# king159/Pair-Net

Hardware: AMD Instinct MI355X
Metric: images/sec (whole node), 100-query 800x1333, 1/2/4/8 MI355X (higher is better)
Workload: dtype f32

## Files before the change

### include/pairnet_hip.h

```cpp
#ifndef PAIRNET_HIP_H_
#define PAIRNET_HIP_H_

#include <stdint.h>

#ifdef __cplusplus
extern "C" {
#endif

#define PN_ABI_VERSION 33
int pn_abi_version(void);

#define PN_GEMM_RELU       1
#define PN_GEMM_A_COLMAJOR 2
#define PN_GEMM_FORCE_TILE 4
#define PN_GEMM_FORCE_SKINNY 8
#define PN_GEMM_FORCE_TILE64 16
#define PN_GEMM_FORCE_TILE128x64 32
#define PN_GEMM_RELU_AFTER_RES 128
#define PN_GEMM_GELU 256
#define PN_GEMM_RESERVE_SHIFT 16
#define PN_GEMM_RESERVE(n) ((((n) / 8) & 0x3ff) << PN_GEMM_RESERVE_SHIFT)
#define PN_GEMM_KSPLIT_SHIFT 26
#define PN_GEMM_KSPLIT(n) (((n) & 31) << PN_GEMM_KSPLIT_SHIFT)

// ... 140 lines not shown
                         int64_t out_bstride, void* stream);
int pn_bilinear_planar_f32(const float* in, float* out, int64_t P, int hi,
                           int wi, int ho, int wo, void* stream);
int pn_bilinear_stencil_rows_f32(const float* in, float* out, int B, int hi, int wi, int ho,
                                 int wo, int C, int64_t in_bstride, int64_t out_bstride,
                                 void* stream);
int pn_bilinear_planar_gt0_u8(const float* in, uint8_t* out, int64_t P, int hi,
                              int wi, int ho, int wo, void* stream);

int pn_mask_pack(const float* logits, uint32_t* bits, int32_t* rowall,
                 int64_t R, int Nk, void* stream);
int pn_mask_pack_stencil(const float* logits4, uint32_t* bits, int32_t* rowall, int64_t R,
                         int hi, int wi, int ho, int wo, void* stream);

int pn_mask_stencil_gemm_f32(const float* me, int64_t ld_me, int64_t stride_me, const float* rows,
                             int64_t ld_rows, int64_t stride_rows, uint32_t* bits,
                             int32_t* rowall, int B, int Q, int Nk, int K, int hi, int wi, int ho,
                             int wo, int flags, void* stream);

int pn_mask_stencil_gather_gemm_f32(const float* me, int64_t ld_me, int64_t stride_me,
                                    const float* mf, int64_t ld_mf, int64_t stride_mf,
                                    uint32_t* bits, int32_t* rowall, int B, int Q, int Nk, int K,
                                    int hi, int wi, int ho, int wo, int flags, void* stream);

int64_t pn_attn_scratch_floats(int B, int Q, int Nk);
int pn_attention_f32(const float* q, int64_t ldq, const float* k, int64_t ldk,
                     const float* v, int64_t ldv, const uint32_t* maskbits,
                     const int32_t* rowall, float* out, int64_t ldo,
                     float* scratch, int B, int Q, int Nk, float scale,
                     void* stream);

int pn_mlearner_first_f32(const float* in, const float* w1, const float* b1,
                          float* out, int B, int S, int C, void* stream);
int pn_ppn_front_f32(const float* sub_embed, const float* obj_embed, const float* w1,
                     const float* b1, float* importance_raw, float* c1, int B, int Q, float eps,
                     void* stream);
int pn_mlearner_last_f32(const float* in, const float* w3, const float* b3,
                         float* out, int B, int S, int C, void* stream);

int pn_topk_pairs(const float* scores, int64_t* idx, int64_t* sub, int64_t* obj,
                  int64_t* pair, int B, int Q, int k, void* stream);
int pn_topk_f32(const float* scores, int64_t* idx, int64_t* quot, int64_t* rem, int B,
                int n, int div, int k, void* stream);
int pn_topk_strided_f32(const float* scores, int64_t elem_stride, int64_t row_stride,
                        int64_t* idx, int64_t* quot, int64_t* rem, int B, int n, int div, int k,
                        void* stream);
// ... 221 lines not shown
```

### pair-net_amd/csrc/gemm.hip

```cpp
#include "common.h"
#include "gemm_common.h"

#ifndef PN_GEMM_WGS64
#define PN_GEMM_WGS64 5
#endif
#ifndef PN_GEMM_WGS128x64
#define PN_GEMM_WGS128x64 3
#endif
#ifndef PN_GEMM_BIGM_128x64
#define PN_GEMM_BIGM_128x64 0
#endif
#ifndef PN_GEMM_WGS64_SPILLING
#define PN_GEMM_WGS64_SPILLING 5
#endif

#ifndef PN_GEMM_LDS2
#define PN_GEMM_LDS2 0
#endif

template <int BM, int BN, int AMODE>
struct TileSmem {
  static constexpr int A_ELEMS = (AMODE == A_COL) ? 32 * (BM + 4) : BM * 36;
  static constexpr int STAGE = A_ELEMS + BN * 36;
  static constexpr int FLOATS = STAGE * (PN_GEMM_LDS2 ? 2 : 1);
// ... 14 lines not shown
  static constexpr int min_waves = (BM * BN <= 64 * 64 && value > 4) ? value : 1;
};

struct TileRef {
  int pi;
  int bz, tm, tn;
};

template <int BM, int BN, int WM, int WN, int AMODE, bool ADD, typename Locator, int EPI = 0>
__device__ __forceinline__ void gemm_persistent(const Locator& loc, const int ntiles,
                                                float* smem) {
  constexpr int BK = 32, LD = BK + 4;
  constexpr int WAVES_N = BN / WN;
  constexpr int TM = WM / 32, TN = WN / 32;
  constexpr int LDK = BM + 4;
  constexpr int A_ELEMS = TileSmem<BM, BN, AMODE>::A_ELEMS;
  constexpr int NT = 64 * (BM / WM) * WAVES_N;
  constexpr int RPP = NT / 8;
  constexpr int NA = (BM * BK / 4) / NT;
  constexpr int NB = (BN * BK / 4) / NT;
  constexpr int QM = BM / 4;
  constexpr int KSTEP = NT / QM;
  static_assert(NT == 128 || NT == 256 || NT == 512, "2, 4 or 8 waves");

  const int xcd = blockIdx.x & 7, slot = blockIdx.x >> 3, per = gridDim.x >> 3;
  const int q8 = ntiles >> 3, r8 = ntiles & 7;
  const int base = (xcd < r8) ? xcd * (q8 + 1) : r8 * (q8 + 1) + (xcd - r8) * q8;
  const int cnt = q8 + (xcd < r8 ? 1 : 0);
  if (slot >= cnt) return;

  const int tid = threadIdx.x, lane = tid & 63, wave = tid >> 6;
  const int li = lane & 31, lh = lane >> 5;
  const int wm = wave / WAVES_N, wn = wave % WAVES_N;
  const int kc = (tid & 7) * 4;
  float* const sA = smem;
  float* const sB = smem + A_ELEMS;

  int lpi = 0, lK = 0, lkt0 = 0;
  const float* bA = nullptr;
  const float* bW = nullptr;
  const float* bAdd = nullptr;
  __amdgpu_buffer_rsrc_t rA = make_rsrc(nullptr), rW = rA, rAdd = rA;
  unsigned a_off[NA], add_off[ADD ? NA : 1], w_off[NB];
  int cy[NA], cx[NA];
  unsigned a_tap[AMODE == A_CONV ? NA : 1];
  unsigned a_off1[AMODE == A_COL ? NA : 1][4];
// ... 21 lines not shown
#pragma unroll
      for (int j = 0; j < NA; ++j) {
        const unsigned krow = (unsigned)(min(tid / QM + KSTEP * j, p.K - 1)) * (unsigned)p.lda;
        a_off[j] = (krow + (unsigned)min(mq, p.M - 1)) * 4u;
#pragma unroll
        for (int e = 0; e < 4; ++e) a_off1[j][e] = (krow + (unsigned)min(mq + e, p.M - 1)) * 4u;
      }
    } else {
#pragma unroll
      for (int j = 0; j < NA; ++j) {
        const int gm = min(m0 + (tid >> 3) + RPP * j, p.M - 1);
        if (AMODE == A_CONV) {
          const int oy = gm / p.Wo, ox = gm - oy * p.Wo;
          cy[j] = oy * p.stride;
          cx[j] = ox * p.stride;
          a_off[j] = ((unsigned)(cy[j] * p.Wd + cx[j]) * (unsigned)p.Cin + kc) * 4u;
        } else {
          a_off[j] = ((unsigned)gm * (unsigned)p.lda + kc) * 4u;
        }
        if (ADD) add_off[j] = ((unsigned)(p.Aadd ? gm % p.aadd_rows : gm) *
                                   (unsigned)(p.Aadd ? p.ldaadd : p.lda) + kc) * 4u;
      }
    }
    if constexpr (EPI == 1 || EPI == 3) {
      const StencilP& st = loc.st;
#pragma unroll
      for (int j = 0; j < NB; ++j) {
        const int c = (tid >> 3) + RPP * j;
        const int key = min(tr.tn * 16 + (c >> 5) * 8 + (c & 7), st.nk - 1);
        if constexpr (EPI == 3) {
          const int t = (c >> 3) & 3;
          const int oy = key / st.wo, ox = key - oy * st.wo;
          const Tap ty = make_tap(oy, st.hi, st.ho), tx = make_tap(ox, st.wi, st.wo);
          const int sy = (t & 2) ? ty.i1 : ty.i0, sx = (t & 1) ? tx.i1 : tx.i0;
          w_off[j] = ((unsigned)(sy * st.wi + sx) * (unsigned)p.ldw + kc) * 4u;
        } else {
          w_off[j] = ((unsigned)(((c >> 3) & 3) * st.nk + key) * (unsigned)p.ldw + kc) * 4u;
        }
      }
    } else {
#pragma unroll
      for (int j = 0; j < NB; ++j)
        w_off[j] = ((unsigned)min(n0 + (tid >> 3) + RPP * j, p.N - 1) * (unsigned)p.ldw + kc) * 4u;
    }
  };

  float4 ra[NA], rad[ADD ? NA : 1], rb[NB];
  bool st_ragged = false, st_add = false;
  int st_k0 = 0;
  unsigned st_in = 0;
  auto load_chunk = [&](int kt) {
    const int k0 = (lkt0 + kt) * BK;
    const bool ragged = k0 + BK > lK;
    st_ragged = ragged;
    st_add = l_add;
    st_k0 = k0;
    if (AMODE == A_COL) {
      const GemmP& p = loc.P(lpi);
      const int soff = (ragged ? 0 : k0) * (int)p.lda * 4;
      if (l_vec) {
// ... 105 lines not shown
      if (AMODE == A_COL) {
        const float* s = fA + (kb * 8) * LDK + mi * 32;
        fa[mi] = make_float4(s[0], s[LDK], s[2 * LDK], s[3 * LDK]);
      } else {
        fa[mi] = ld4(fA + mi * 32 * LD + kb * 8);
      }
    }
#pragma unroll
    for (int ni = 0; ni < TN; ++ni) fb[ni] = ld4(fB + ni * 32 * LD + kb * 8);
  };
  auto compute = [&]() {
    float4 fa[2][TM], fb[2][TN];
    read_frag(0, fa[0], fb[0]);
#pragma unroll
    for (int kb = 0; kb < BK / 8; ++kb) {
      const int cur = kb & 1;
      if (kb + 1 < BK / 8) read_frag(kb + 1, fa[cur ^ 1], fb[cur ^ 1]);
#pragma unroll
      for (int t = 0; t < 4; ++t)
#pragma unroll
        for (int mi = 0; mi < TM; ++mi)
#pragma unroll
          for (int ni = 0; ni < TN; ++ni) {
            const float4 av = fa[cur][mi], bv = fb[cur][ni];
            acc[mi][ni] = mfma32(t == 0 ? av.x : t == 1 ? av.y : t == 2 ? av.z : av.w,
                                 t == 0 ? bv.x : t == 1 ? bv.y : t == 2 ? bv.z : bv.w,
                                 acc[mi][ni]);
          }
    }
  };

  static_assert(EPI != 2 || (TM == 1 && TN == 1 && !PN_GEMM_LDS2), "two-phase mode: 32x32 waves, one LDS stage");
  float keep[EPI == 2 ? 16 : 1];
  TileRef cur = loc(base + slot);
  set_tile(cur);
  load_chunk(0);
#if PN_GEMM_LDS2
  constexpr int STAGE = TileSmem<BM, BN, AMODE>::STAGE;
  int wso = 0;
  {
    const GemmP& p0 = loc.P(cur.pi);
    int nk0 = (p0.K + BK - 1) / BK;
    if (p0.ksplit > 1) nk0 = min(p0.split_chunks, nk0 - (cur.bz % p0.ksplit) * p0.split_chunks);
    store_chunk(0);
    wso = STAGE;
    if (nk0 > 1) {
      load_chunk(1);
// ... 35 lines not shown
          load_chunk(1);
        } else {
          set_tile(loc(base + min(t + 2 * per, cnt - 1)));
          load_chunk(0);
        }
      }
      compute();
      __syncthreads();
      rso = wso;
      wso = STAGE - wso;
    }
#else
    for (int kt = 0; kt < nk; ++kt) {
      __syncthreads();
      store_chunk();
      __syncthreads();
      const bool last = kt + 1 == nk;
      if (last) set_tile(nxt);
      load_chunk(last ? 0 : kt + 1);
      compute();
    }
#endif
    const int m0 = cur.tm * BM, n0 = cur.tn * BN;
    if constexpr (EPI == 1 || EPI == 3) {
      const StencilP& st = loc.st;
      static_assert((EPI != 1 && EPI != 3) || (TM == 1 && TN == 1 && BN == 64), "stencil mode: 64x64 tiles of 32x32 waves");
      const int pl = li & 7;
      const int key0 = cur.tn * 16 + wn * 8;
      const int key = key0 + pl;
      const bool kvalid = key < st.nk;
      const int kk = min(key, st.nk - 1);
      const int oy = kk / st.wo, ox = kk - oy * st.wo;
      const Tap ty = make_tap(oy, st.hi, st.ho), tx = make_tap(ox, st.wi, st.wo);
      const int src = (lane & 32) | pl;
      const int nwords = (st.nk + 31) / 32;
      const int nvalid = min(max(st.nk - key0, 0), 8);
      const unsigned vm = (1u << nvalid) - 1u;
      const int rbase = m0 + wm * WM;
      const bool writer = li == 0;
      const bool last_tile = (cur.tn + 1) * 16 >= st.nk && wn == WAVES_N - 1;
#pragma unroll
      for (int r = 0; r < 16; ++r) {
        const float a = acc[0][0][r];
        const float v00 = __shfl(a, src, 64), v01 = __shfl(a, src + 8, 64);
        const float v10 = __shfl(a, src + 16, 64), v11 = __shfl(a, src + 24, 64);
        const float res = tap_blend(ty, tx, v00, v01, v10, v11);
// ... 101 lines not shown
  const StencilP& st;
  int mt, nt;
  __device__ __forceinline__ const GemmP& P(int) const { return p; }
  __device__ __forceinline__ TileRef operator()(int T) const {
    const int per_b = mt * nt;
    const int bz = T / per_b, r = T - bz * per_b;
    const int tm = r / nt;
    return TileRef{0, bz, tm, r - tm * nt};
  }
};

__global__ __launch_bounds__(256, (TileWgs<64, 64, A_ROW, false>::min_waves))
void k_gemm_stencil(const GemmP p, const StencilP st, const int batch) {
  __shared__ __attribute__((aligned(16))) float smem[TileSmem<64, 64, A_ROW>::FLOATS];
  const StencilLocator loc{p, st, (p.M + 63) / 64, (p.N + 63) / 64};
  gemm_persistent<64, 64, 32, 32, A_ROW, false, StencilLocator, 1>(loc, loc.mt * loc.nt * batch, smem);
}

__global__ __launch_bounds__(256, (TileWgs<64, 64, A_ROW, false>::min_waves))
void k_gemm_stencil_gather(const GemmP p, const StencilP st, const int batch) {
  __shared__ __attribute__((aligned(16))) float smem[TileSmem<64, 64, A_ROW>::FLOATS];
  const StencilLocator loc{p, st, (p.M + 63) / 64, (p.N + 63) / 64};
  gemm_persistent<64, 64, 32, 32, A_ROW, false, StencilLocator, 3>(loc, loc.mt * loc.nt * batch, smem);
}

#define PN_GEMM_WGS_PROJ PN_GEMM_WGS64
struct ProjLocator {
  const GemmP& p;
  const GemmP& sc;
  int mt, nt;
  __device__ __forceinline__ const GemmP& P(int phase) const { return phase ? p : sc; }
  __device__ __forceinline__ TileRef operator()(int T) const {
    const int per_b = mt * nt;
    const int bz = T / per_b, r = T - bz * per_b;
    const int tm = r / nt;
    return TileRef{0, bz, tm, r - tm * nt};
  }
};

__global__ __launch_bounds__(256, PN_GEMM_WGS_PROJ)
void k_gemm_proj(const GemmP p, const GemmP sc, const int batch) {
  __shared__ __attribute__((aligned(16))) float smem[TileSmem<64, 64, A_CONV>::FLOATS];
  const ProjLocator loc{p, sc, (p.M + 63) / 64, (p.N + 63) / 64};
  gemm_persistent<64, 64, 32, 32, A_CONV, false, ProjLocator, 2>(loc, loc.mt * loc.nt * batch, smem);
}

// ... 456 lines not shown
  if (fused) {
    GemmP both = p3;
    both.K = Cin + planes;
    fused = splitk_factor(both, B, splitk_scratch, splitk_scratch_floats, &cps, flags) <= 1;
  }
  if (!fused) {
    if (!idt) return PN_BAD_ARG;
    if (stride == 1) {
      if (int rc = pn_gemm_f32(&ds, stream)) return rc;
    } else if (int rc = pn_conv2d_nhwc_ex_f32(x, Wsc, bsc, nullptr, idt, B, H, W, Cin, Cout, 1, 1,
                                              stride, 0, flags, splitk_scratch,
                                              splitk_scratch_floats, stream)) {
      return rc;
    }
    return pn_gemm_f32(&d3, stream);
  }
  const int64_t ntiles = (int64_t)pn_cdiv((int)M, 64) * pn_cdiv(Cout, 64) * B;
  static const int wgs = resident_wgs(k_gemm_proj, PN_GEMM_WGS_PROJ, 256);
  hipLaunchKernelGGL(k_gemm_proj, dim3(persistent_grid(ntiles, wgs, flags)), dim3(256), 0, s, p3,
                     psc, B);
  return PN_LAUNCH_CHECK();
}

extern "C" int pn_mask_stencil_gemm_f32(const float* me, int64_t ld_me, int64_t stride_me,
                                        const float* rows, int64_t ld_rows, int64_t stride_rows,
                                        uint32_t* bits, int32_t* rowall, int B, int Q, int Nk,
                                        int K, int hi, int wi, int ho, int wo, int flags,
                                        void* stream) {
  if (!me || !rows || !bits || !rowall || B <= 0 || Q <= 0 || Nk <= 0 || K <= 0 || K % 32)
    return PN_BAD_ARG;
  if (hi <= 0 || wi <= 0 || ho <= 0 || wo <= 0 || (int64_t)ho * wo != Nk) return PN_BAD_ARG;
  if (ld_me % 4 || ld_rows % 4 || stride_me % 4 || stride_rows % 4 || !aligned16(me) || !aligned16(rows))
    return PN_BAD_ARG;
  const int64_t lim = (int64_t)1 << 29;
  if ((int64_t)(Q - 1) * ld_me + K >= lim || ((int64_t)4 * Nk - 1) * ld_rows + K >= lim)
    return PN_BAD_ARG;
  GemmP p{};
  p.A = me; p.W = rows; p.lda = ld_me; p.ldw = ld_rows; p.sA = stride_me; p.sW = stride_rows;
  p.M = Q; p.K = K; p.aadd_rows = 1;
  p.N = pn_cdiv(Nk, 16) * 64;
  const StencilP st{bits, rowall, Nk, hi, wi, ho, wo};
  hipStream_t s = (hipStream_t)stream;
  hipLaunchKernelGGL(k_fill_i32, dim3(pn_cdiv(B * Q, 256)), dim3(256), 0, s, rowall, 1, B * Q);
  const int64_t ntiles = (int64_t)pn_cdiv(Q, 64) * (p.N / 64) * B;
  static const int wgs = resident_wgs(k_gemm_stencil, TileWgs<64, 64, A_ROW, false>::value, 256);
  hipLaunchKernelGGL(k_gemm_stencil, dim3(persistent_grid(ntiles, wgs, flags)), dim3(256), 0, s, p, st, B);
  return PN_LAUNCH_CHECK();
}

extern "C" int pn_mask_stencil_gather_gemm_f32(const float* me, int64_t ld_me, int64_t stride_me,
                                               const float* mf, int64_t ld_mf, int64_t stride_mf,
                                               uint32_t* bits, int32_t* rowall, int B, int Q,
                                               int Nk, int K, int hi, int wi, int ho, int wo,
                                               int flags, void* stream) {
  if (!me || !mf || !bits || !rowall || B <= 0 || Q <= 0 || Nk <= 0 || K <= 0 || K % 32)
    return PN_BAD_ARG;
  if (hi <= 0 || wi <= 0 || ho <= 0 || wo <= 0 || (int64_t)ho * wo != Nk) return PN_BAD_ARG;
  if (ld_me % 4 || ld_mf % 4 || stride_me % 4 || stride_mf % 4 || !aligned16(me) || !aligned16(mf))
    return PN_BAD_ARG;
  const int64_t lim = (int64_t)1 << 29;
  if ((int64_t)(Q - 1) * ld_me + K >= lim || ((int64_t)hi * wi - 1) * ld_mf + K >= lim)
    return PN_BAD_ARG;
  GemmP p{};
  p.A = me; p.W = mf; p.lda = ld_me; p.ldw = ld_mf; p.sA = stride_me; p.sW = stride_mf;
  p.M = Q; p.K = K; p.aadd_rows = 1;
  p.N = pn_cdiv(Nk, 16) * 64;
  const StencilP st{bits, rowall, Nk, hi, wi, ho, wo};
  hipStream_t s = (hipStream_t)stream;
  hipLaunchKernelGGL(k_fill_i32, dim3(pn_cdiv(B * Q, 256)), dim3(256), 0, s, rowall, 1, B * Q);
  const int64_t ntiles = (int64_t)pn_cdiv(Q, 64) * (p.N / 64) * B;
  static const int wgs = resident_wgs(k_gemm_stencil_gather, TileWgs<64, 64, A_ROW, false>::value, 256);
  hipLaunchKernelGGL(k_gemm_stencil_gather, dim3(persistent_grid(ntiles, wgs, flags)), dim3(256), 0,
                     s, p, st, B);
  return PN_LAUNCH_CHECK();
}

extern "C" int pn_abi_version(void) { return PN_ABI_VERSION; }
```

### pair-net_amd/head.py

```python
import math
from collections import OrderedDict

import torch

from . import hip
from . import plans
from .plans import Arena, PlanCache, measure_bytes
from .config import ConfigDict

INSTANCE_OFFSET = 1000


def _decoder_param_shapes(prefix, num_layers, ffn_dim, out):
    for i in range(num_layers):
        p = "%s.layers.%d." % (prefix, i)
        for a in (0, 1):
            out[p + "attentions.%d.attn.in_proj_weight" % a] = (768, 256)
            out[p + "attentions.%d.attn.in_proj_bias" % a] = (768,)
            out[p + "attentions.%d.attn.out_proj.weight" % a] = (256, 256)
            out[p + "attentions.%d.attn.out_proj.bias" % a] = (256,)
        out[p + "ffns.0.layers.0.0.weight"] = (ffn_dim, 256)
        out[p + "ffns.0.layers.0.0.bias"] = (ffn_dim,)
        out[p + "ffns.0.layers.1.weight"] = (256, ffn_dim)
        out[p + "ffns.0.layers.1.bias"] = (256,)
# ... 79 lines not shown
                                                 transformer_decoder=transformer_decoder,
                                                 relation_decoder=relation_decoder))
        self.other_drop_rates.pop("relation_decoder.transformerlayers.ffn_cfgs.ffn_drop", None)
        self.test_cfg, self.train_cfg = test_cfg, train_cfg
        assert len(self.in_channels) == 4 and num_transformer_feat_level == 3
        assert num_obj_query <= 256 and num_rel_query <= 128
        self._params = OrderedDict(
            (k, torch.zeros(s)) for k, s in self.param_shapes().items())
        self.device = None
        self.w = None
        self._plans = PlanCache()
        self._arenas, self._post_arenas, self._consts, self._pe = {}, {}, {}, OrderedDict()
        self._dummies = {}
        self._post = OrderedDict()
        self._pan_jobs = []
        self.graph_after = 1
        self.exact_mask_order = True
        self.conv_algo = "winograd4"
        self.use_graphs = False
        self.grid_reserve = 0
        self.fuse_ppn_front = True
        self.fuse_mask_pack = True
        self.gather_mask_stencil = True
        self.fuse_lateral_upadd = False
        self.enc_fused_ln = ("proj", "ffn")
        self.group_input_convs = False
        self.gemm_arithmetic = "bf16x3"
        self.msda_s3_out = False
        self.init_weights()

    def param_shapes(self):
        s = OrderedDict()
        Q, R = self.num_obj_query, self.num_rel_query
        _decoder_param_shapes("relation_decoder", self.num_rel_layers, self.rel_ffn, s)
        s["rel_query_embed.weight"] = (R, 256)
        s["rel_query_embed2.weight"] = (2 * R, 256)
        s["rel_query_embed3.weight"] = (2 * R, 256)
        s["rel_query_feat.weight"] = (R, 256)
        for i, (ci, co) in enumerate(((1, 64), (64, 64), (64, 1))):
            s["update_importance.conv_layers.%d.0.weight" % i] = (co, ci, 7, 7)
            s["update_importance.conv_layers.%d.0.bias" % i] = (co,)
        pd = "pixel_decoder."
        for i in range(3):
            cin = self.in_channels[3 - i]
            s[pd + "input_convs.%d.conv.weight" % i] = (256, cin, 1, 1)
            s[pd + "input_convs.%d.conv.bias" % i] = (256,)
# ... 538 lines not shown
                 batch=pl.B, sA=Q * 256, sW=pl.HW2 * 256, sC=Q * pl.HW2)

    def _head_embed(self, q, pl, with_cls, full_mask, cls_out=None, mp_out=None, normed=False):
        w, B, Q = self.w, pl.B, self.num_obj_query
        cls_out = pl.cls if cls_out is None else cls_out
        mp_out = pl.MP if mp_out is None else mp_out
        if not normed:
            hip.layernorm(q, w["transformer_decoder.post_norm.weight"],
                          w["transformer_decoder.post_norm.bias"], pl.qn)
        if with_cls:
            hip.linear(pl.qn, w["cls_embed.weight"], w["cls_embed.bias"], cls_out.view(B * Q, -1))
        self._mlp3("mask_embed", pl.qn, pl.me, pl)
        if full_mask:
            self._mask_logits(pl.me, pl, mp_out)

    def _attn_mask(self, pl, lvl, mp=None, me=None):
        B, Q = pl.B, self.num_obj_query
        h, wd = pl.shapes[lvl]
        n = h * wd
        if self.exact_mask_order == "full":
            hip.bilinear_planar(pl.MP if mp is None else mp, pl.ML, B * Q, pl.hw2[0], pl.hw2[1],
                                h, wd)
        elif self.exact_mask_order and self.fuse_mask_pack:
            if self._gathers_stencil():
                hip.mask_stencil_gather_gemm(pl.me if me is None else me, pl.MF, pl.bits,
                                             pl.rowall, B, Q, pl.hw2[0], pl.hw2[1], h, wd)
            else:
                hip.mask_stencil_gemm(pl.me if me is None else me, pl.MFs[lvl], pl.bits,
                                      pl.rowall, B, Q, pl.hw2[0], pl.hw2[1], h, wd)
            return
        elif self.exact_mask_order:
            hip.gemm(pl.me if me is None else me, pl.MFs[lvl], pl.ML4, M=Q, N=4 * n, K=256,
                     lda=256, ldw=256, ldc=4 * n, batch=B, sA=Q * 256, sW=4 * n * 256,
                     sC=Q * 4 * n, force="tile64")
            hip.mask_pack_stencil(pl.ML4, pl.bits, pl.rowall, B * Q, pl.hw2[0], pl.hw2[1], h, wd)
            return
        else:
            hip.gemm(pl.me if me is None else me, pl.MFd[lvl], pl.ML, M=Q, N=n, K=256, lda=256,
                     ldw=256, ldc=n, batch=B, sA=Q * 256, sW=n * 256, sC=Q * n)
        hip.mask_pack(pl.ML, pl.bits, pl.rowall, B * Q, n)

    def _layer(self, pre, x, xpos, x1, x2, y, Qp, VQK, att, hbuf, Kp, ldk, Vp, ldv, Nk, B, nq,
               bits, rowall, scr, ffn, self_first=False, post=None, x_in=None):
        w = self.w
        scale = 1.0 / math.sqrt(32.0)
        ac = pre + "attentions.%d.attn." % (1 if self_first else 0)
        as_ = pre + "attentions.%d.attn." % (0 if self_first else 1)
        nc, ns = ("norms.1.", "norms.0.") if self_first else ("norms.0.", "norms.1.")

        def cross(src, dst):
            hip.linear(src, w[ac + "in_proj_weight"][:256], w[ac + "in_proj_bias"][:256], Qp,
                       aadd=xpos)
# ... 142 lines not shown
    def _check_feats(self, feats, img_metas):
        pv = getattr(self, "_packed_version", None)
        if self.w is not None and pv is not None and pv != self._weights_version():
            self._drop_weight_state()
        B = len(img_metas)
        assert len(feats) == 4 and all(f.shape[0] == B for f in feats)
        nchw = all(f.is_contiguous() for f in feats)
        nhwc = not nchw and all(f.is_contiguous(memory_format=torch.channels_last) for f in feats)
        for f, c in zip(feats, self.in_channels):
            if not f.is_cuda or f.dtype != torch.float32 or f.shape[1] != c or not (nchw or nhwc):
                raise RuntimeError("feats must be fp32 [B,C,H,W] device tensors with channels %s, "
                                   "all contiguous or all in channels_last memory format"
                                   % self.in_channels)
        if self.device is None:
            self.to(feats[0].device)
        shapes = [tuple(feats[3 - l].shape[-2:]) for l in range(3)]
        self._feats_nhwc = nhwc
        return B, shapes, tuple(feats[0].shape[-2:])

    def _run_stage(self, which, pl, feats=None):
        cfg = (self.exact_mask_order, self.conv_algo, self.fuse_ppn_front, self.grid_reserve,
               tuple(self.enc_fused_ln), self.group_input_convs,
               getattr(self, "fuse_mask_pack", True), self.gemm_arithmetic, self.msda_s3_out,
               getattr(self, "gather_mask_stencil", True), getattr(self, "fuse_lateral_upadd", False))
        if pl.graph_cfg != cfg:
            pl.graph_a = pl.graph_b = None
            pl.graphs_a = OrderedDict()
            pl.graph_c = PlanCache(self.POST_VIEWS)
            pl.graph_cfg = cfg
        cur = torch.cuda.current_stream(self.device)
        pl.streams[cur.cuda_stream] = cur
        try:
            self._run_stage_on(which, pl, feats, cur)
        finally:
            plans.note_use(cur)

    def _run_stage_on(self, which, pl, feats, cur):
        if which == "a":
            if not pl.pe_waited:
                if pl.pe_ready.query():
                    pl.pe_waited = True
                else:
                    cur.wait_event(pl.pe_ready)
            ptrs = tuple(f.data_ptr() for f in feats)
            ent = pl.graphs_a.get(ptrs)
            if ent is None:
# ... 323 lines not shown
```

### pair-net_amd/hip.py

```python
import contextlib
import ctypes as C
import os
import threading

import torch

from .build import LIB_PATH

LIB_PATH = os.environ.get("PAIRNET_LIB") or LIB_PATH

_i32, _i64, _f32, _vp = C.c_int32, C.c_int64, C.c_float, C.c_void_p

GEMM_RELU, GEMM_A_COLMAJOR, GEMM_FORCE_TILE, GEMM_FORCE_SKINNY = 1, 2, 4, 8
GEMM_GELU = 256
GEMM_FORCE_TILE64, GEMM_FORCE_TILE128x64 = 16, 32
GEMM_RELU_AFTER_RES = 128
GEMM_GROUP_MAX = 18


class GemmDesc(C.Structure):
    _fields_ = [("A", _vp), ("lda", _i64), ("strideA", _i64),
                ("Aadd", _vp), ("ldaadd", _i64), ("aadd_rows", _i32),
                ("aadd_from_col", _i32),
                ("W", _vp), ("ldw", _i64), ("strideW", _i64),
# ... 105 lines not shown
    "pn_window_attention_bwd_f32": (C.c_int, [_vp, _i64, _vp, _vp, _vp, _i64, _vp, _i64, _vp, _i64, _vp]
                                    + [_i32] * 7 + [_f32, _vp]),
    "pn_grad_norm_clip_f32": (C.c_int, [_vp, _i64, _f32, _f32, _vp, _vp, _vp]),
    "pn_adamw_f32": (C.c_int, [_vp, _vp, _vp, _vp, _i64, _vp, _vp, _vp, _i32, _f32, _f32, _f32, _f32,
                               _f32, _i32, _vp, _f32, _vp]),
    "pn_adamw_guarded_f32": (C.c_int, [_vp, _vp, _vp, _vp, _i64, _vp, _vp, _vp, _i32, _f32, _f32,
                                       _f32, _f32, _f32, _i32, _vp, _f32, _vp, _vp]),
    "pn_lsa_f32": (C.c_int, [_vp, _i64, _vp, _i32, _i64, _vp, _vp, _i64, _vp, _vp]),
    "pn_loss_targets": (C.c_int, [_vp] * 6 + [_i64, _i32, _i32, _i32, _i32] + [_vp] * 5),
    "pn_msda_loc_f32": (C.c_int, [_vp, _i64, _vp, _vp, _vp, _vp, _vp, _i32, _i32, _i32, _i32, _vp]),
    "pn_msda_bwd_f32": (C.c_int, [_vp, _i64] + [_vp] * 8 + [_i32, _i32, _i32, _i32, _vp]),
    "pn_gather_probe_f32": (C.c_int, [_vp, _vp, _vp, _i32, _i32, _vp]),
    "pn_sine_pe_f32": (C.c_int, [_vp, _vp, _i32, _i32, _i32, _f32, _vp]),
    "pn_sine_pe_offset_f32": (C.c_int, [_vp, _vp, _i32, _i32, _i32, _f32, _f32, _vp]),
    "pn_bilinear_nhwc_f32": (C.c_int, [_vp, _vp] + [_i32] * 7 + [_i64, _i64, _vp]),
    "pn_bilinear_planar_f32": (C.c_int, [_vp, _vp, _i64] + [_i32] * 4 + [_vp]),
    "pn_bilinear_planar_gt0_u8": (C.c_int, [_vp, _vp, _i64] + [_i32] * 4 + [_vp]),
    "pn_mask_pack": (C.c_int, [_vp, _vp, _vp, _i64, _i32, _vp]),
    "pn_mask_pack_stencil": (C.c_int, [_vp, _vp, _vp, _i64, _i32, _i32, _i32, _i32, _vp]),
    "pn_mask_stencil_gemm_f32": (C.c_int, [_vp, _i64, _i64, _vp, _i64, _i64, _vp, _vp] +
                                 [_i32] * 9 + [_vp]),
    "pn_mask_stencil_gather_gemm_f32": (C.c_int, [_vp, _i64, _i64, _vp, _i64, _i64, _vp, _vp] +
                                        [_i32] * 9 + [_vp]),
    "pn_bilinear_stencil_rows_f32": (C.c_int, [_vp, _vp] + [_i32] * 6 + [_i64, _i64, _vp]),
    "pn_attn_scratch_floats": (_i64, [_i32, _i32, _i32]),
    "pn_attention_f32": (C.c_int, [_vp, _i64, _vp, _i64, _vp, _i64, _vp, _vp, _vp,
                                   _i64, _vp, _i32, _i32, _i32, _f32, _vp]),
    "pn_ppn_front_f32": (C.c_int, [_vp] * 6 + [_i32, _i32, _f32, _vp]),
    "pn_mlearner_first_f32": (C.c_int, [_vp, _vp, _vp, _vp, _i32, _i32, _i32, _vp]),
    "pn_mlearner_last_f32": (C.c_int, [_vp, _vp, _vp, _vp, _i32, _i32, _i32, _vp]),
    "pn_topk_pairs": (C.c_int, [_vp, _vp, _vp, _vp, _vp, _i32, _i32, _i32, _vp]),
    "pn_topk_f32": (C.c_int, [_vp, _vp, _vp, _vp, _i32, _i32, _i32, _i32, _vp]),
    "pn_topk_strided_f32": (C.c_int, [_vp, _i64, _i64, _vp, _vp, _vp, _i32, _i32, _i32, _i32, _vp]),
    "pn_gather_rows_f32": (C.c_int, [_vp, _vp, _vp, _i32, _i32, _i32, _i64, _vp]),
    "pn_cls_argmax_f32": (C.c_int, [_vp, _vp, _vp, _i64, _i32, _i32, _vp]),
    "pn_rel_dists_f32": (C.c_int, [_vp, _vp, _i64, _i32, _vp]),
    "pn_softmax_fg_f32": (C.c_int, [_vp, _vp, _vp, _i64, _i32, _vp]),
    "pn_row_argmax_f32": (C.c_int, [_vp, _vp, _i64, _i32, _vp]),
    "pn_triplet_finish": (C.c_int, [_vp] * 9 + [_i32, _i32, _vp]),
    "pn_panoptic_f32": (C.c_int, [_vp, _vp, _vp, _vp, _vp, _i32, _i64, _vp]),
    "pn_panoptic_state_bytes": (_i64, []),
    "pn_panoptic_device_f32": (C.c_int, [_vp, _vp, _vp] + [_i32] * 6 + [_vp, _vp, _vp, _vp,
                                                                        _i32, _vp]),
    "pn_panoptic_continue_f32": (C.c_int, [_vp, _vp, _vp, _vp, _i32, _i32, _i32, _vp]),
    "pn_pack_triplets_f32": (C.c_int, [_vp] * 5 + [_i32, _i32, _vp]),
    "pn_copy_stream": (C.c_int, [_vp, _vp, _i64, _i32, _vp]),
# ... 585 lines not shown


def bilinear_planar(x, out, P, hi, wi, ho, wo):
    _check(lib().pn_bilinear_planar_f32(_ptr(x), _ptr(out), P, hi, wi, ho, wo, _stream()),
           "pn_bilinear_planar_f32")


def bilinear_planar_gt0(x, out, P, hi, wi, ho, wo):
    _check(lib().pn_bilinear_planar_gt0_u8(_ptr(x), _ptr(out, torch.uint8), P, hi, wi, ho,
                                           wo, _stream()), "pn_bilinear_planar_gt0_u8")


def mask_pack(logits, bits, rowall, R, Nk):
    _check(lib().pn_mask_pack(_ptr(logits), _ptr(bits, torch.int32),
                              _ptr(rowall, torch.int32), R, Nk, _stream()), "pn_mask_pack")


def mask_pack_stencil(logits4, bits, rowall, R, hi, wi, ho, wo):
    _check(lib().pn_mask_pack_stencil(_ptr(logits4), _ptr(bits, torch.int32),
                                      _ptr(rowall, torch.int32), R, hi, wi, ho, wo, _stream()),
           "pn_mask_pack_stencil")


def mask_stencil_gemm(me, rows, bits, rowall, B, Q, hi, wi, ho, wo, K=256):
    Nk = ho * wo
    _check(_launch("k_gemm_stencil", 2.0 * B * Q * 4 * Nk * K,
                   4.0 * B * (Q * K + 4 * Nk * K) + B * Q * Nk / 8.0,
                   lambda: lib().pn_mask_stencil_gemm_f32(
                       _ptr(me), me.stride(0), Q * me.stride(0), _ptr(rows), rows.stride(-2),
                       rows.stride(0) if rows.dim() == 3 else 4 * Nk * rows.stride(-2),
                       _ptr(bits, torch.int32), _ptr(rowall, torch.int32), B, Q, Nk, K, hi, wi,
                       ho, wo, _reserve_flag(), _stream()),
                   meta=(Q, 4 * Nk, K, B, False)), "pn_mask_stencil_gemm_f32")


def mask_stencil_gather_gemm(me, mf, bits, rowall, B, Q, hi, wi, ho, wo, K=256):
    Nk = ho * wo
    _check(_launch("k_gemm_stencil_gather", 2.0 * B * Q * 4 * Nk * K,
                   4.0 * B * (Q * K + 4 * Nk * K) + B * Q * Nk / 8.0,
                   lambda: lib().pn_mask_stencil_gather_gemm_f32(
                       _ptr(me), me.stride(0), Q * me.stride(0), _ptr(mf), mf.stride(-2),
                       mf.stride(0) if mf.dim() == 3 else hi * wi * mf.stride(-2),
                       _ptr(bits, torch.int32), _ptr(rowall, torch.int32), B, Q, Nk, K, hi, wi,
                       ho, wo, _reserve_flag(), _stream()),
                   meta=(Q, 4 * Nk, K, B, False)), "pn_mask_stencil_gather_gemm_f32")


def bilinear_stencil_rows(x, out, B, hi, wi, ho, wo, Cc, in_bstride, out_bstride):
    _check(lib().pn_bilinear_stencil_rows_f32(_ptr(x), _ptr(out), B, hi, wi, ho, wo, Cc,
                                              in_bstride, out_bstride, _stream()),
           "pn_bilinear_stencil_rows_f32")


def attn_scratch_floats(B, Q, Nk):
    return lib().pn_attn_scratch_floats(B, Q, Nk)


def attention(q, ldq, k, ldk, v, ldv, bits, rowall, out, ldo, scratch, B, Q, Nk, scale):
    _check(_launch("k_attn_chunk", 8.0 * B * 8 * Q * Nk * 32 / 2,
                   4.0 * B * 256 * (2 * Q + 2 * Nk),
# ... 603 lines not shown
```

Baseline: 224.3.

## Blend stencil mask taps in MFMA registers by swapping operands and tap layout

Adds register-resident stencil kernels (EPI 4/5) for the mask-logit GEMM. The four bilinear taps of each output pixel are interleaved along N and the MFMA operands are swapped, so each lane's accumulator already holds all four taps of a pixel. The blend-and-threshold then runs directly on the accumulators and bits are written per byte, skipping the shared-memory epilogue of the old stencil path. It is enabled by default through a new head flag. The risks are correctness of the new tap and key mapping and its per-byte bit writes.

```diff
diff --git a/include/pairnet_hip.h b/include/pairnet_hip.h
--- a/include/pairnet_hip.h
+++ b/include/pairnet_hip.h
@@ -186,6 +186,16 @@
                                     const float* mf, int64_t ld_mf, int64_t stride_mf,
                                     uint32_t* bits, int32_t* rowall, int B, int Q, int Nk, int K,
                                     int hi, int wi, int ho, int wo, int flags, void* stream);
+
+int pn_mask_stencil_regs_gemm_f32(const float* me, int64_t ld_me, int64_t stride_me,
+                                  const float* rows, int64_t ld_rows, int64_t stride_rows,
+                                  uint32_t* bits, int32_t* rowall, int B, int Q, int Nk, int K,
+                                  int hi, int wi, int ho, int wo, int flags, void* stream);
+int pn_mask_stencil_regs_gather_gemm_f32(const float* me, int64_t ld_me, int64_t stride_me,
+                                         const float* mf, int64_t ld_mf, int64_t stride_mf,
+                                         uint32_t* bits, int32_t* rowall, int B, int Q, int Nk,
+                                         int K, int hi, int wi, int ho, int wo, int flags,
+                                         void* stream);
 
 int64_t pn_attn_scratch_floats(int B, int Q, int Nk);
 int pn_attention_f32(const float* q, int64_t ldq, const float* k, int64_t ldk,
diff --git a/pair-net_amd/csrc/gemm.hip b/pair-net_amd/csrc/gemm.hip
--- a/pair-net_amd/csrc/gemm.hip
+++ b/pair-net_amd/csrc/gemm.hip
@@ -60,6 +60,9 @@
   constexpr int QM = BM / 4;
   constexpr int KSTEP = NT / QM;
   static_assert(NT == 128 || NT == 256 || NT == 512, "2, 4 or 8 waves");
+  constexpr bool STENCIL_REGS = EPI == 4 || EPI == 5;
+  constexpr bool STENCIL_GATHER = EPI == 3 || EPI == 5;
+  constexpr bool STENCIL = EPI == 1 || EPI == 3 || STENCIL_REGS;
 
   const int xcd = blockIdx.x & 7, slot = blockIdx.x >> 3, per = gridDim.x >> 3;
   const int q8 = ntiles >> 3, r8 = ntiles & 7;
@@ -127,20 +130,21 @@
                                    (unsigned)(p.Aadd ? p.ldaadd : p.lda) + kc) * 4u;
       }
     }
-    if constexpr (EPI == 1 || EPI == 3) {
+    if constexpr (STENCIL) {
       const StencilP& st = loc.st;
 #pragma unroll
       for (int j = 0; j < NB; ++j) {
         const int c = (tid >> 3) + RPP * j;
-        const int key = min(tr.tn * 16 + (c >> 5) * 8 + (c & 7), st.nk - 1);
-        if constexpr (EPI == 3) {
-          const int t = (c >> 3) & 3;
+        const int t = STENCIL_REGS ? (c & 3) : ((c >> 3) & 3);
+        const int key = min(tr.tn * 16 + (c >> 5) * 8 + (STENCIL_REGS ? (c & 31) >> 2 : (c & 7)),
+                            st.nk - 1);
+        if constexpr (STENCIL_GATHER) {
           const int oy = key / st.wo, ox = key - oy * st.wo;
           const Tap ty = make_tap(oy, st.hi, st.ho), tx = make_tap(ox, st.wi, st.wo);
           const int sy = (t & 2) ? ty.i1 : ty.i0, sx = (t & 1) ? tx.i1 : tx.i0;
           w_off[j] = ((unsigned)(sy * st.wi + sx) * (unsigned)p.ldw + kc) * 4u;
         } else {
-          w_off[j] = ((unsigned)(((c >> 3) & 3) * st.nk + key) * (unsigned)p.ldw + kc) * 4u;
+          w_off[j] = ((unsigned)(t * st.nk + key) * (unsigned)p.ldw + kc) * 4u;
         }
       }
     } else {
@@ -292,7 +296,8 @@
         for (int mi = 0; mi < TM; ++mi)
 #pragma unroll
           for (int ni = 0; ni < TN; ++ni) {
-            const float4 av = fa[cur][mi], bv = fb[cur][ni];
+            const float4 av = STENCIL_REGS ? fb[cur][ni] : fa[cur][mi];
+            const float4 bv = STENCIL_REGS ? fa[cur][mi] : fb[cur][ni];
             acc[mi][ni] = mfma32(t == 0 ? av.x : t == 1 ? av.y : t == 2 ? av.z : av.w,
                                  t == 0 ? bv.x : t == 1 ? bv.y : t == 2 ? bv.z : bv.w,
                                  acc[mi][ni]);
@@ -374,6 +379,41 @@
     }
 #endif
     const int m0 = cur.tm * BM, n0 = cur.tn * BN;
+    if constexpr (STENCIL_REGS) {
+      const StencilP& st = loc.st;
+      static_assert(!STENCIL_REGS || (TM == 1 && TN == 1 && BN == 64), "stencil mode: 64x64 tiles of 32x32 waves");
+      const int key0 = cur.tn * 16 + wn * 8;
+      int oy = (key0 + lh) / st.wo, ox = (key0 + lh) - oy * st.wo;
+      unsigned nib = 0;
+#pragma unroll
+      for (int g = 0; g < 4; ++g) {
+        const Tap ty = make_tap(oy, st.hi, st.ho), tx = make_tap(ox, st.wi, st.wo);
+        const float res = tap_blend(ty, tx, acc[0][0][4 * g], acc[0][0][4 * g + 1],
+                                    acc[0][0][4 * g + 2], acc[0][0][4 * g + 3]);
+        const bool kvalid = key0 + 2 * g + lh < st.nk;
+        nib |= (kvalid && res < 0.f) ? 1u << (2 * g + lh) : 0u;
+#pragma unroll
+        for (int e = 0; e < 2; ++e)
+          if (++ox == st.wo) { ox = 0; ++oy; }
+      }
+      const unsigned byte = nib | (unsigned)__shfl_xor((int)nib, 32, 64);
+      const int nwords = (st.nk + 31) / 32;
+      const int nvalid = min(max(st.nk - key0, 0), 8);
+      const unsigned vm = (1u << nvalid) - 1u;
+      const int row = m0 + wm * WM + li;
+      const bool last_tile = (cur.tn + 1) * 16 >= st.nk && wn == WAVES_N - 1;
+      if (lh == 0 && row < p.M) {
+        const int64_t grow = (int64_t)cur.bz * p.M + row;
+        unsigned char* bp = reinterpret_cast<unsigned char*>(st.bits + grow * nwords);
+        bp[cur.tn * 2 + wn] = (unsigned char)byte;
+        if (last_tile)
+          for (int e = cur.tn * 2 + wn + 1; e < nwords * 4; ++e) bp[e] = 0;
+        if (~byte & vm) st.rowall[grow] = 0;
+      }
+      cur = nxt;
+      t += per;
+      continue;
+    }
     if constexpr (EPI == 1 || EPI == 3) {
       const StencilP& st = loc.st;
       static_assert((EPI != 1 && EPI != 3) || (TM == 1 && TN == 1 && BN == 64), "stencil mode: 64x64 tiles of 32x32 waves");
@@ -521,6 +561,20 @@
   __shared__ __attribute__((aligned(16))) float smem[TileSmem<64, 64, A_ROW>::FLOATS];
   const StencilLocator loc{p, st, (p.M + 63) / 64, (p.N + 63) / 64};
   gemm_persistent<64, 64, 32, 32, A_ROW, false, StencilLocator, 3>(loc, loc.mt * loc.nt * batch, smem);
+}
+
+__global__ __launch_bounds__(256, (TileWgs<64, 64, A_ROW, false>::min_waves))
+void k_stencil_regs(const GemmP p, const StencilP st, const int batch) {
+  __shared__ __attribute__((aligned(16))) float smem[TileSmem<64, 64, A_ROW>::FLOATS];
+  const StencilLocator loc{p, st, (p.M + 63) / 64, (p.N + 63) / 64};
+  gemm_persistent<64, 64, 32, 32, A_ROW, false, StencilLocator, 4>(loc, loc.mt * loc.nt * batch, smem);
+}
+
+__global__ __launch_bounds__(256, (TileWgs<64, 64, A_ROW, false>::min_waves))
+void k_stencil_regs_gather(const GemmP p, const StencilP st, const int batch) {
+  __shared__ __attribute__((aligned(16))) float smem[TileSmem<64, 64, A_ROW>::FLOATS];
+  const StencilLocator loc{p, st, (p.M + 63) / 64, (p.N + 63) / 64};
+  gemm_persistent<64, 64, 32, 32, A_ROW, false, StencilLocator, 5>(loc, loc.mt * loc.nt * batch, smem);
 }
 
 #define PN_GEMM_WGS_PROJ PN_GEMM_WGS64
@@ -1023,57 +1077,57 @@
   return PN_LAUNCH_CHECK();
 }
 
-extern "C" int pn_mask_stencil_gemm_f32(const float* me, int64_t ld_me, int64_t stride_me,
-                                        const float* rows, int64_t ld_rows, int64_t stride_rows,
-                                        uint32_t* bits, int32_t* rowall, int B, int Q, int Nk,
-                                        int K, int hi, int wi, int ho, int wo, int flags,
-                                        void* stream) {
-  if (!me || !rows || !bits || !rowall || B <= 0 || Q <= 0 || Nk <= 0 || K <= 0 || K % 32)
+template <void (*KERN)(GemmP, StencilP, int)>
+static int launch_stencil(const float* me, int64_t ld_me, int64_t stride_me,
+                          const float* w, int64_t ld_w, int64_t stride_w, int64_t w_rows,
+                          uint32_t* bits, int32_t* rowall, int B, int Q, int Nk, int K, int hi,
+                          int wi, int ho, int wo, int flags, void* stream) {
+  if (!me || !w || !bits || !rowall || B <= 0 || Q <= 0 || Nk <= 0 || K <= 0 || K % 32)
     return PN_BAD_ARG;
   if (hi <= 0 || wi <= 0 || ho <= 0 || wo <= 0 || (int64_t)ho * wo != Nk) return PN_BAD_ARG;
-  if (ld_me % 4 || ld_rows % 4 || stride_me % 4 || stride_rows % 4 || !aligned16(me) || !aligned16(rows))
+  if (ld_me % 4 || ld_w % 4 || stride_me % 4 || stride_w % 4 || !aligned16(me) || !aligned16(w))
     return PN_BAD_ARG;
   const int64_t lim = (int64_t)1 << 29;
-  if ((int64_t)(Q - 1) * ld_me + K >= lim || ((int64_t)4 * Nk - 1) * ld_rows + K >= lim)
-    return PN_BAD_ARG;
+  if ((int64_t)(Q - 1) * ld_me + K >= lim || (w_rows - 1) * ld_w + K >= lim) return PN_BAD_ARG;
   GemmP p{};
-  p.A = me; p.W = rows; p.lda = ld_me; p.ldw = ld_rows; p.sA = stride_me; p.sW = stride_rows;
+  p.A = me; p.W = w; p.lda = ld_me; p.ldw = ld_w; p.sA = stride_me; p.sW = stride_w;
   p.M = Q; p.K = K; p.aadd_rows = 1;
   p.N = pn_cdiv(Nk, 16) * 64;
   const StencilP st{bits, rowall, Nk, hi, wi, ho, wo};
   hipStream_t s = (hipStream_t)stream;
   hipLaunchKernelGGL(k_fill_i32, dim3(pn_cdiv(B * Q, 256)), dim3(256), 0, s, rowall, 1, B * Q);
   const int64_t ntiles = (int64_t)pn_cdiv(Q, 64) * (p.N / 64) * B;
-  static const int wgs = resident_wgs(k_gemm_stencil, TileWgs<64, 64, A_ROW, false>::value, 256);
-  hipLaunchKernelGGL(k_gemm_stencil, dim3(persistent_grid(ntiles, wgs, flags)), dim3(256), 0, s, p, st, B);
+  static const int wgs = resident_wgs(KERN, TileWgs<64, 64, A_ROW, false>::value, 256);
+  hipLaunchKernelGGL(KERN, dim3(persistent_grid(ntiles, wgs, flags)), dim3(256), 0, s, p, st, B);
   return PN_LAUNCH_CHECK();
 }
 
+extern "C" int pn_mask_stencil_gemm_f32(const float* me, int64_t ld_me, int64_t stride_me,
+               const float* rows, int64_t ld_rows, int64_t stride_rows, uint32_t* bits, int32_t* rowall, int B, int Q,
+               int Nk, int K, int hi, int wi, int ho, int wo, int flags, void* stream) {
+  return launch_stencil<k_gemm_stencil>(me, ld_me, stride_me, rows, ld_rows, stride_rows, (int64_t)4 * Nk,
+                        bits, rowall, B, Q, Nk, K, hi, wi, ho, wo, flags, stream);
+}
+
 extern "C" int pn_mask_stencil_gather_gemm_f32(const float* me, int64_t ld_me, int64_t stride_me,
-                                               const float* mf, int64_t ld_mf, int64_t stride_mf,
-                                               uint32_t* bits, int32_t* rowall, int B, int Q,
-                                               int Nk, int K, int hi, int wi, int ho, int wo,
-                                               int flags, void* stream) {
-  if (!me || !mf || !bits || !rowall || B <= 0 || Q <= 0 || Nk <= 0 || K <= 0 || K % 32)
-    return PN_BAD_ARG;
-  if (hi <= 0 || wi <= 0 || ho <= 0 || wo <= 0 || (int64_t)ho * wo != Nk) return PN_BAD_ARG;
-  if (ld_me % 4 || ld_mf % 4 || stride_me % 4 || stride_mf % 4 || !aligned16(me) || !aligned16(mf))
-    return PN_BAD_ARG;
-  const int64_t lim = (int64_t)1 << 29;
-  if ((int64_t)(Q - 1) * ld_me + K >= lim || ((int64_t)hi * wi - 1) * ld_mf + K >= lim)
-    return PN_BAD_ARG;
-  GemmP p{};
-  p.A = me; p.W = mf; p.lda = ld_me; p.ldw = ld_mf; p.sA = stride_me; p.sW = stride_mf;
-  p.M = Q; p.K = K; p.aadd_rows = 1;
-  p.N = pn_cdiv(Nk, 16) * 64;
-  const StencilP st{bits, rowall, Nk, hi, wi, ho, wo};
-  hipStream_t s = (hipStream_t)stream;
-  hipLaunchKernelGGL(k_fill_i32, dim3(pn_cdiv(B * Q, 256)), dim3(256), 0, s, rowall, 1, B * Q);
-  const int64_t ntiles = (int64_t)pn_cdiv(Q, 64) * (p.N / 64) * B;
-  static const int wgs = resident_wgs(k_gemm_stencil_gather, TileWgs<64, 64, A_ROW, false>::value, 256);
-  hipLaunchKernelGGL(k_gemm_stencil_gather, dim3(persistent_grid(ntiles, wgs, flags)), dim3(256), 0,
-                     s, p, st, B);
-  return PN_LAUNCH_CHECK();
+               const float* mf, int64_t ld_mf, int64_t stride_mf, uint32_t* bits, int32_t* rowall, int B, int Q,
+               int Nk, int K, int hi, int wi, int ho, int wo, int flags, void* stream) {
+  return launch_stencil<k_gemm_stencil_gather>(me, ld_me, stride_me, mf, ld_mf, stride_mf, (int64_t)hi * wi,
+                        bits, rowall, B, Q, Nk, K, hi, wi, ho, wo, flags, stream);
+}
+
+extern "C" int pn_mask_stencil_regs_gemm_f32(const float* me, int64_t ld_me, int64_t stride_me,
+               const float* rows, int64_t ld_rows, int64_t stride_rows, uint32_t* bits, int32_t* rowall, int B, int Q,
+               int Nk, int K, int hi, int wi, int ho, int wo, int flags, void* stream) {
+  return launch_stencil<k_stencil_regs>(me, ld_me, stride_me, rows, ld_rows, stride_rows, (int64_t)4 * Nk,
+                        bits, rowall, B, Q, Nk, K, hi, wi, ho, wo, flags, stream);
+}
+
+extern "C" int pn_mask_stencil_regs_gather_gemm_f32(const float* me, int64_t ld_me, int64_t stride_me,
+               const float* mf, int64_t ld_mf, int64_t stride_mf, uint32_t* bits, int32_t* rowall, int B, int Q,
+               int Nk, int K, int hi, int wi, int ho, int wo, int flags, void* stream) {
+  return launch_stencil<k_stencil_regs_gather>(me, ld_me, stride_me, mf, ld_mf, stride_mf, (int64_t)hi * wi,
+                        bits, rowall, B, Q, Nk, K, hi, wi, ho, wo, flags, stream);
 }
 
 extern "C" int pn_abi_version(void) { return PN_ABI_VERSION; }
diff --git a/pair-net_amd/head.py b/pair-net_amd/head.py
--- a/pair-net_amd/head.py
+++ b/pair-net_amd/head.py
@@ -125,6 +125,7 @@
         self.fuse_ppn_front = True
         self.fuse_mask_pack = True
         self.gather_mask_stencil = True
+        self.mask_blend_in_registers = 1
         self.fuse_lateral_upadd = False
         self.enc_fused_ln = ("proj", "ffn")
         self.group_input_convs = False
@@ -709,12 +710,14 @@
             hip.bilinear_planar(pl.MP if mp is None else mp, pl.ML, B * Q, pl.hw2[0], pl.hw2[1],
                                 h, wd)
         elif self.exact_mask_order and self.fuse_mask_pack:
+            regs = bool(getattr(self, "mask_blend_in_registers", 1))
             if self._gathers_stencil():
                 hip.mask_stencil_gather_gemm(pl.me if me is None else me, pl.MF, pl.bits,
-                                             pl.rowall, B, Q, pl.hw2[0], pl.hw2[1], h, wd)
+                                             pl.rowall, B, Q, pl.hw2[0], pl.hw2[1], h, wd,
+                                             regs=regs)
             else:
                 hip.mask_stencil_gemm(pl.me if me is None else me, pl.MFs[lvl], pl.bits,
-                                      pl.rowall, B, Q, pl.hw2[0], pl.hw2[1], h, wd)
+                                      pl.rowall, B, Q, pl.hw2[0], pl.hw2[1], h, wd, regs=regs)
             return
         elif self.exact_mask_order:
             hip.gemm(pl.me if me is None else me, pl.MFs[lvl], pl.ML4, M=Q, N=4 * n, K=256,
@@ -903,6 +906,7 @@
         cfg = (self.exact_mask_order, self.conv_algo, self.fuse_ppn_front, self.grid_reserve,
                tuple(self.enc_fused_ln), self.group_input_convs,
                getattr(self, "fuse_mask_pack", True), self.gemm_arithmetic, self.msda_s3_out,
+               getattr(self, "mask_blend_in_registers", 1),
                getattr(self, "gather_mask_stencil", True), getattr(self, "fuse_lateral_upadd", False))
         if pl.graph_cfg != cfg:
             pl.graph_a = pl.graph_b = None
diff --git a/pair-net_amd/hip.py b/pair-net_amd/hip.py
--- a/pair-net_amd/hip.py
+++ b/pair-net_amd/hip.py
@@ -151,6 +151,10 @@
                                  [_i32] * 9 + [_vp]),
     "pn_mask_stencil_gather_gemm_f32": (C.c_int, [_vp, _i64, _i64, _vp, _i64, _i64, _vp, _vp] +
                                         [_i32] * 9 + [_vp]),
+    "pn_mask_stencil_regs_gemm_f32": (C.c_int, [_vp, _i64, _i64, _vp, _i64, _i64, _vp, _vp] +
+                                      [_i32] * 9 + [_vp]),
+    "pn_mask_stencil_regs_gather_gemm_f32": (C.c_int, [_vp, _i64, _i64, _vp, _i64, _i64, _vp, _vp] +
+                                             [_i32] * 9 + [_vp]),
     "pn_bilinear_stencil_rows_f32": (C.c_int, [_vp, _vp] + [_i32] * 6 + [_i64, _i64, _vp]),
     "pn_attn_scratch_floats": (_i64, [_i32, _i32, _i32]),
     "pn_attention_f32": (C.c_int, [_vp, _i64, _vp, _i64, _vp, _i64, _vp, _vp, _vp,
@@ -782,8 +786,18 @@
            "pn_mask_pack_stencil")
 
 
-def mask_stencil_gemm(me, rows, bits, rowall, B, Q, hi, wi, ho, wo, K=256):
+def mask_stencil_gemm(me, rows, bits, rowall, B, Q, hi, wi, ho, wo, K=256, regs=False):
     Nk = ho * wo
+    if regs:
+        _check(_launch("k_gemm_stencil_regs", 2.0 * B * Q * 4 * Nk * K,
+                       4.0 * B * (Q * K + 4 * Nk * K) + B * Q * Nk / 8.0,
+                       lambda: lib().pn_mask_stencil_regs_gemm_f32(
+                           _ptr(me), me.stride(0), Q * me.stride(0), _ptr(rows), rows.stride(-2),
+                           rows.stride(0) if rows.dim() == 3 else 4 * Nk * rows.stride(-2),
+                           _ptr(bits, torch.int32), _ptr(rowall, torch.int32), B, Q, Nk, K, hi, wi,
+                           ho, wo, _reserve_flag(), _stream()),
+                       meta=(Q, 4 * Nk, K, B, False)), "pn_mask_stencil_regs_gemm_f32")
+        return
     _check(_launch("k_gemm_stencil", 2.0 * B * Q * 4 * Nk * K,
                    4.0 * B * (Q * K + 4 * Nk * K) + B * Q * Nk / 8.0,
                    lambda: lib().pn_mask_stencil_gemm_f32(
@@ -794,8 +808,18 @@
                    meta=(Q, 4 * Nk, K, B, False)), "pn_mask_stencil_gemm_f32")
 
 
-def mask_stencil_gather_gemm(me, mf, bits, rowall, B, Q, hi, wi, ho, wo, K=256):
+def mask_stencil_gather_gemm(me, mf, bits, rowall, B, Q, hi, wi, ho, wo, K=256, regs=False):
     Nk = ho * wo
+    if regs:
+        _check(_launch("k_gemm_stencil_regs_gather", 2.0 * B * Q * 4 * Nk * K,
+                       4.0 * B * (Q * K + 4 * Nk * K) + B * Q * Nk / 8.0,
+                       lambda: lib().pn_mask_stencil_regs_gather_gemm_f32(
+                           _ptr(me), me.stride(0), Q * me.stride(0), _ptr(mf), mf.stride(-2),
+                           mf.stride(0) if mf.dim() == 3 else hi * wi * mf.stride(-2),
+                           _ptr(bits, torch.int32), _ptr(rowall, torch.int32), B, Q, Nk, K, hi, wi,
+                           ho, wo, _reserve_flag(), _stream()),
+                       meta=(Q, 4 * Nk, K, B, False)), "pn_mask_stencil_regs_gather_gemm_f32")
+        return
     _check(_launch("k_gemm_stencil_gather", 2.0 * B * Q * 4 * Nk * K,
                    4.0 * B * (Q * K + 4 * Nk * K) + B * Q * Nk / 8.0,
                    lambda: lib().pn_mask_stencil_gather_gemm_f32(
```

After: 225.5, median of 6. Within noise of the previous version (+0.5%).
